# ToyotaResearchInstitute/idto

Hardware: AMD Instinct MI355X
Metric: Gauss-Newton iters/sec (grad+Hessian+solve), mini_cheetah N=40 (higher is better)
Workload: dtype f64; 1 GPU; mini_cheetah (nq=19, nv=18, 9 contact pairs), horizon N=40, dt=0.05, forward differences, one Gauss-Newton iteration per step; parallelism=single GPU

## Files before the change

### idto_amd/csrc/penta_pipe.h

```cpp
#pragma once

#include "kernels.h"
#include "penta_nd.h"
#include "solver_layout.h"

namespace idto_dev {


enum {
  PF_SLOTGEN = 0,
  PF_SLOTGEN2 = 3,
  PF_ROWDONE = 6,
  PF_ROWDONE2 = 9,
  PF_STAGED = 12,
  PF_INITD = 14,
  PF_INITD2 = 16,
  PF_GDONE = 18,
  PF_COPIED = 22,
  PF_COPIED2 = 25,
  PF_ABORT = 28,
  PF_JOINED = 29,
  PF_HIDONE = 30,
  PF_HIDONE2 = 31,
  PF_T0 = 40,
// ... 102 lines not shown
    }
  }
  if constexpr (J + 1 < K) {
    const double m1 = rdlane(t, J + 1);
    xr[J + 1] = __builtin_fma(-m1, xj, xr[J + 1]);
  }
  if constexpr (J == JH) hook();
  if constexpr (J >= 1) {
#pragma unroll
    for (int r = J + 2; r < K; ++r) xr[r] = __builtin_fma(-mu_p[r], xj_p, xr[r]);
    if constexpr ((J & 1) == 0 && J + 1 < K) asm volatile("" ::"v"(mu_p[J]));
  }
  __builtin_amdgcn_sched_barrier(0);
  if constexpr (J + 1 < K) pipe_pivot<K, J + 1, JH>(xr, inv_next, mu, xj, rowp, rawp, slot0, is63, hook, dbg);
}

template <int K, int J, int JH, class Hook, class Need>
__device__ __forceinline__ void pipe_spike_pivot(double (&xr)[K], const double (&mu_p)[K], const double xj_p, const double m1,
                                                 double* __restrict__ rowp, double* __restrict__ fout, const bool store,
                                                 const double* __restrict__ arow, Hook hook, Need need) {
  using G = PipeGeo<K>;
  if constexpr (J == JH) hook();
  if constexpr (J + 2 < K) need(J + 2);
  const double xj = xr[J];
  if constexpr (J + 1 < K) {
    if constexpr (J >= 1) xr[J + 1] = __builtin_fma(-mu_p[J + 1], xj_p, xr[J + 1]);
    xr[J + 1] = __builtin_fma(-m1, xj, xr[J + 1]);
  }
  rowp[J * G::RS] = pipe_setlane<63>(xj, 0x3ff00000, 0);
  __atomic_signal_fence(__ATOMIC_SEQ_CST);
  if (store) __hip_atomic_store(fout + J, xj, __ATOMIC_RELAXED, __HIP_MEMORY_SCOPE_AGENT);
  double mu[K];
  double m1n = 0.0;
  if constexpr (J + 2 < K) {
    const double2* p2 = reinterpret_cast<const double2*>(arow + J * G::RS);
#pragma unroll
    for (int m = (J + 2) / 2; m < (K + 1) / 2; ++m) {
      const double2 v = p2[m];
      mu[2 * m] = v.x;
      if (2 * m + 1 < K) mu[2 * m + 1] = v.y;
    }
    m1n = arow[(J + 1) * G::RS + J + 2];
  }
  if constexpr (J >= 1) {
#pragma unroll
    for (int r = J + 2; r < K; ++r) xr[r] = __builtin_fma(-mu_p[r], xj_p, xr[r]);
  }
  __builtin_amdgcn_sched_barrier(0);
  if constexpr (J + 1 < K) pipe_spike_pivot<K, J + 1, JH>(xr, mu, xj, m1n, rowp, fout, store, arow, hook, need);
}

template <int K>
__device__ __forceinline__ void pipe_read_mult(const double* __restrict__ row, int pos0, double (&mu)[K]) {
  const double2* p2 = reinterpret_cast<const double2*>(row + pos0);
#pragma unroll
  for (int m = 0; m < K / 2; ++m) { const double2 v = p2[m]; mu[2 * m] = v.x; mu[2 * m + 1] = v.y; }
  if (K & 1) mu[K - 1] = row[pos0 + K - 1];
}

__device__ __forceinline__ void pipe_wait_row(const PipeCtl& c, const double* word) {
  pipe_lds_int* hi = (pipe_lds_int*)word + 1;
  int n = 0;
  while ((__builtin_amdgcn_readfirstlane(*hi) & 0x7ff80000) == 0x7ff80000) {
    __builtin_amdgcn_s_sleep(1);
    if (pipe_giveup(c, ++n)) break;
  }
  __atomic_signal_fence(__ATOMIC_SEQ_CST);
}

struct PipeArgs {
  int n, k;
  const double* HA; const double* HB; const double* HC; const double* b;
  double rhs_sign;
  double* x;
  double* Ust; double* Hst; double* Est; double* Dst;
  double* xch; unsigned* flags; unsigned epoch;
  unsigned* status; unsigned fact_id;
  double* fst; int fstride; unsigned long long* frowcnt;
  double* wst;
  double* xjoin_ll;
  double* join_ll;
  const unsigned* asm_ready; int asm_first, asm_rows;
  double* ts;
};

struct PipeAsm {
  int on;
  int nq, nv, rows, first;
  DevProblem P;
  const double* q; const double* terms; const double* v_res; const double* nplus;
  double* g; double* HA; double* HB; double* HC;
  AltSel alt;
  unsigned* ready;
  const double* gate;
  int decide;
  const double* dq;
  const double* dv; const double* dslab; int dslab_stride; double* dcost; int ddiag;
  TrDecideArgs dT; AltSel dalt;
  double* dword; unsigned depoch;
  double* g2; double* HA2; double* HB2; double* HC2;
  const double* curpre;
};
template <bool DEC = false>
__device__ __forceinline__ bool pipe_asm_on(const PipeAsm& F, size_t o, const SpinCtl sc = SpinCtl{nullptr, 0}, int* cur = nullptr) {
  if (!F.on) return false;
  if (DEC && F.decide) {
    double x = 0.0;
    if ((threadIdx.x & 63) == 0) {
      const double* word = at_problem(F.dword, o);
      if (!spin_wait([&] { return tr_ll_try(word, F.depoch, x); }, sc)) x = 1.0;
    }
    const int code = __builtin_amdgcn_readfirstlane((int)x) - 1;
    if (cur) *cur = code >> 1;
    return (code & 1) != 0;
  }
  return !(F.gate && *at_problem(F.gate, o) == 0.0);
}

__device__ __forceinline__ void pipe_decide_role(const PipeAsm& F, const size_t pstride) {
  const size_t o = (size_t)blockIdx.y * pstride, w = o + (size_t)alt_offset(F.dalt, o);
  const DevProblem P = at_problem(F.P, o);
  TrDecideArgs T = F.dT;
  T.state = at_problem(T.state, o); T.out = at_problem(T.out, o); T.q = at_problem(T.q, o);
  T.q_trial = at_problem(T.q_trial, o); T.rows += (size_t)blockIdx.y * T.rows_stride;
  T.part2 = at_problem(T.part2, o);
  if (T.lambda) T.lambda = at_problem(T.lambda, o);
  const double cur_old = T.state[TRS_CUR];
  const bool acc = cost_body<4>(F.nq, F.nv, P, at_problem(F.dq, o), at_problem(F.dv, w), at_problem(F.dslab, w), F.dslab_stride,
                             at_problem(F.dcost, o), F.ddiag, nullptr, nullptr, T);
  if (threadIdx.x == 0) {
    const int cur_new = acc ? (cur_old != 0.0 ? 0 : 1) : (cur_old != 0.0 ? 1 : 0);
    tr_ll_store(at_problem(F.dword, o), (double)(1 + (acc ? 1 : 0) + 2 * cur_new), F.depoch);
  }
}

template <bool DEC = false>
__device__ __forceinline__ void pipe_assemble(double* ts, const unsigned epoch, const size_t pstride, PipeAsm F, const int first_wg,
                                              const SpinCtl sc = SpinCtl{nullptr, 0}) {
  struct { double* ts; unsigned epoch; size_t pstride; } A{ts, epoch, pstride};
  extern __shared__ double lds[];
  const bool decided = DEC && F.decide;
  const int a0 = (int)blockIdx.x - first_wg;
  if (decided && a0 == 0) { pipe_decide_role(F, pstride); return; }
  const int a = decided ? a0 - 1 : a0, i = a >> 2, part = a & 3;
  if (i >= F.rows) return;
  const size_t o = (size_t)blockIdx.y * A.pstride;
  if (!decided && !pipe_asm_on<false>(F, o)) return;
  if (A.ts && threadIdx.x == 0)
    atomicMax(reinterpret_cast<unsigned long long*>(A.ts + first_wg * 64 + 1), (unsigned long long)__double_as_longlong((double)wall_clock64()));
  if (A.ts && a == 4 && threadIdx.x == 0) A.ts[first_wg * 64 + 8] = (double)wall_clock64();
  const size_t w = o + (size_t)(decided ? (((*at_problem(F.curpre, o) != 0.0) != (F.dalt.which != 0)) ? F.dalt.off : 0) : alt_offset(F.alt, o));
  const DevProblem P = at_problem(F.P, o);
  const double* qa = at_problem(decided ? F.dq : F.q, o);
  assemble_terms_row<true>(F.nq, F.nv, P, qa, at_problem(F.terms, w), at_problem(F.v_res, w), at_problem(F.nplus, w),
                           at_problem(decided ? F.g2 : F.g, o), at_problem(decided ? F.HA2 : F.HA, o),
                           at_problem(decided ? F.HB2 : F.HB, o), at_problem(decided ? F.HC2 : F.HC, o), i, part, lds);
  if (A.ts && a == 4 && threadIdx.x == 0) A.ts[first_wg * 64 + 9] = (double)wall_clock64();
  asm volatile("s_waitcnt vmcnt(0)" ::: "memory");
  __syncthreads();
  if (A.ts && a == 4 && threadIdx.x == 0) A.ts[first_wg * 64 + 10] = (double)wall_clock64();
  if (threadIdx.x == 0)
    __hip_atomic_store(at_problem(F.ready, o) + 4 * i + part, A.epoch, __ATOMIC_RELAXED, __HIP_MEMORY_SCOPE_AGENT);
  if (A.ts && threadIdx.x == 0)
    atomicMax(reinterpret_cast<unsigned long long*>(A.ts + first_wg * 64), (unsigned long long)__double_as_longlong((double)wall_clock64()));
  if (decided) {
    if (!pipe_asm_on<true>(F, o, sc)) return;
// ... 562 lines not shown
    for (int t = 0; t < nloc; ++t) {
      const int slot = t % 3;
      const double* row0 = ring + slot * G::SLOT;
      const bool prod = t + 2 < nrows;
      if (!prod && SPK) {
        pipe_wait(ctl, PF_SLOTGEN + slot, t + 1);
        PipeWatch<K, false> watch(row0, true);
        double* xout = (lane >> 2) == 0 ? A.Dst + (size_t)orig(t) * K : A.fst + (size_t)t * A.fstride + 2 * K * ks;
#pragma unroll
        for (int sq = 0; sq < SK; ++sq) {
          watch.need(ctl, (4 * sq + 3 < K ? 4 * sq + 3 : K - 1));
          const int r = 4 * sq + xr4;
          if (lane < 8 && r < K) __hip_atomic_store(xout + r, row0[r * RS + xpos], __ATOMIC_RELAXED, __HIP_MEMORY_SCOPE_AGENT);
        }
      }
      if (prod) {
        pipe_wait(ctl, PF_SLOTGEN + slot, t + 1);
        if (SPK) pipe_wait(ctl, PF_SLOTGEN2 + slot, t + 1);
        PipeWatch<K, SPK> watch(row0, true);
        double* xout = !SPK ? nullptr : (lane >> 2) == 0 ? A.Dst + (size_t)orig(t) * K : A.fst + (size_t)t * A.fstride + 2 * K * ks;
        d4 acc[CT][TT];
#pragma unroll
        for (int tc = 0; tc < CT; ++tc)
#pragma unroll
          for (int tr = 0; tr < TT; ++tr) acc[tc][tr] = d4{0.0, 0.0, 0.0, 0.0};
#pragma unroll
        for (int sq = 0; sq < SK; ++sq) {
          watch.need(ctl, (4 * sq + 3 < K ? 4 * sq + 3 : K - 1));
          if (SPK) {
            const int r = 4 * sq + xr4;
            if (lane < 8 && r < K) __hip_atomic_store(xout + r, row0[r * RS + xpos], __ATOMIC_RELAXED, __HIP_MEMORY_SCOPE_AGENT);
          }
          const double* row = row0 + (4 * sq + fk) * RS;
          double a[TT], bq[CT];
#pragma unroll
          for (int tr = 0; tr < TT; ++tr) a[tr] = row[G::oE + 16 * tr + fl];
#pragma unroll
          for (int tc = 0; tc < CT; ++tc) {
            const int ci = 16 * tc + fl;
            bq[tc] = row[ci < G::KE + 2 ? G::oRE + ci : G::oF + ci - (G::KE + 2)];
          }
#pragma unroll
          for (int tc = 0; tc < CT; ++tc)
#pragma unroll
            for (int tr = 0; tr < TT; ++tr) acc[tc][tr] = __builtin_amdgcn_mfma_f64_16x16x4f64(a[tr], bq[tc], acc[tc][tr], 0, 0, 0);
        }
        double* gout = gbuf + (t & 1) * G::NGC * GS;
#pragma unroll
        for (int tc = 0; tc < CT; ++tc)
#pragma unroll
          for (int tr = 0; tr < TT; ++tr)
#pragma unroll
            for (int rg = 0; rg < 4; ++rg) {
              const int r = 16 * tr + fk + 4 * rg, ci = 16 * tc + fl;
              if (r < K && ci < NCG) gout[ci * GS + r] = acc[tc][tr][rg];
            }
        pipe_post(ctl, PF_GDONE + (t & 1), t + 1);
      }
      if (SPK) {
        asm volatile("s_waitcnt vmcnt(0)" ::: "memory");
        if (lane == 0) __hip_atomic_fetch_add(A.frowcnt + t, 2ull, __ATOMIC_RELAXED, __HIP_MEMORY_SCOPE_AGENT);
      }
    }
  }
  __syncthreads();
  if (tid == 0 && ctl.f[PF_ABORT] != 0 && cfg.spin.word) {
    __hip_atomic_store(cfg.spin.word, cfg.spin.id, __ATOMIC_RELAXED, __HIP_MEMORY_SCOPE_SYSTEM);
    __hip_atomic_fetch_add(cfg.spin.word + 1, 1u, __ATOMIC_RELAXED, __HIP_MEMORY_SCOPE_SYSTEM);
  }
  chain_ts(cfg, 2);
}


__device__ __forceinline__ double pipe_half_sum(double v) {
  const unsigned lo = (unsigned)__double2loint(v), hi = (unsigned)__double2hiint(v);
  const auto a = __builtin_amdgcn_permlane32_swap(lo, lo, false, false);
  const auto b = __builtin_amdgcn_permlane32_swap(hi, hi, false, false);
  return __hiloint2double((int)b[0], (int)a[0]) + __hiloint2double((int)b[1], (int)a[1]);
}

template <int K, bool SPK>
__device__ __forceinline__ bool pipe_backward_fits(const PipeLds& L, int nloc) { return nloc * PipeBack<K, SPK>::BS + 4 * PipeBack<K, SPK>::KE + 2 <= L.xall; }

template <int K, bool SPK, bool WGLOB = false>
__device__ __forceinline__ void pipe_backward(const PipeArgs& A, const ChainCfg& cfg, const PipeLds& L) {
  extern __shared__ double lds[];
  using B = PipeBack<K, SPK && !WGLOB>;
  constexpr int ks = ldl_ks(K), KE = B::KE, YS = B::YS, KS2 = K * ks;
  const int tid = threadIdx.x, lane = tid & 63, wave = __builtin_amdgcn_readfirstlane(tid >> 6), nwaves = blockDim.x >> 6;
  const bool mirror = cfg.mirror != 0, producer = cfg.producer != 0;
  const int nloc = cfg.nloc, m_split = cfg.m_split, k = A.k;
  auto orig = [&](int il) { const int o = mirror ? cfg.base - il : cfg.base + il; return o < 0 ? 0 : o; };
  double* xb = lds + nloc * B::BS;
  double* dump = xb + 4 * KE;
  auto solve = [&](const double* Us, double (&xr)[K]) __attribute__((always_inline)) {
    constexpr int NP = (K + 1) / 2;
    double2 ub[2][NP];
    auto loadu = [&](int r, double2 (&u)[NP]) __attribute__((always_inline)) {
      const double2* u2 = reinterpret_cast<const double2*>(Us + r * ks);
#pragma unroll
      for (int m = (r + 1) / 2; m < NP; ++m) u[m] = u2[m];
    };
    if (K >= 2) loadu(K - 2, ub[0]);
#pragma unroll
    for (int q = 0; q < K - 1; ++q) {
      const int r = K - 2 - q;
      if (r >= 1) loadu(r - 1, ub[(q + 1) & 1]);
      asm volatile("" ::: "memory");
      double a0 = 0.0, a1 = 0.0;
#pragma unroll
      for (int m = (r + 1) / 2; m < NP; ++m) {
        const double2 u = ub[q & 1][m];
        if (2 * m > r) a0 = __builtin_fma(u.x, xr[2 * m], a0);
        if (2 * m + 1 < K) a1 = __builtin_fma(u.y, xr[2 * m + 1], a1);
      }
      xr[r] -= a0 + a1;
    }
  };
  auto do_pass = [&](const int il, const int pass, const bool stage) __attribute__((always_inline)) {
    const bool partner = WGLOB && pass == 1;
    if (partner) {
      spin_wait([&] { return __hip_atomic_load(cfg.wp_frowcnt + il, __ATOMIC_RELAXED, __HIP_MEMORY_SCOPE_AGENT) >= cfg.frowtarget; }, cfg.spin);
      (void)__hip_atomic_load(cfg.wp_frowcnt + il, __ATOMIC_ACQUIRE, __HIP_MEMORY_SCOPE_AGENT);
    }
    const int op = cfg.wp_mirror ? cfg.wp_base - il : cfg.wp_base + il;
    const int o = partner ? (op < 0 ? 0 : op) : orig(il);
    double* slot = lds + il * B::BS;
    double* Us = partner ? lds + L.W + 2 * KE + 2 + wave * KS2 : slot + ((pass && !WGLOB) ? B::oW : B::oYZ);
    constexpr int NU = (KS2 + 63) / 64;
    double uv[NU];
    if (stage) {
#pragma unroll
      for (int t = 0; t < NU; ++t) uv[t] = A.Ust[(size_t)o * KS2 + (lane + 64 * t < KS2 ? lane + 64 * t : 0)];
    }
    const double dinv = (lane < K) ? A.Dst[(size_t)o * K + lane] : 0.0;
    double xr[K];
    double* dst = dump;
    int dstride = 0;
    if (pass == 0) {
      const double* src = (lane < K) ? A.Hst + (size_t)o * KS2 + lane : A.Est + (size_t)o * KS2 + (lane < 2 * K ? lane - K : 0);
      const double mg = lane < 2 * K ? 1.0 : 0.0, mc = lane == 2 * K ? 1.0 : 0.0;
#pragma unroll
      for (int r = 0; r < K; ++r) xr[r] = src[r * ks] * mg + (rdlane(dinv, r) * lds[L.xall + (il + 2) * ks + r]) * mc;
      if (lane < 2 * K) { dst = slot + B::oYZ + (lane < K ? lane : KE + lane - K); dstride = YS; }
      else if (lane == 2 * K) { dst = slot + B::oC; dstride = 1; }
      else if ((K & 1) && lane <= 2 * K + 2) { dst = slot + B::oYZ + (lane == 2 * K + 1 ? K : KE + K); dstride = YS; }
    } else {
      const double* fsrc = (WGLOB ? cfg.wp_fst : A.fst) + (size_t)il * A.fstride + (size_t)(lane < 2 * K ? lane : 0) * ks;
      const double mf = lane < 2 * K ? 1.0 : 0.0;
#pragma unroll
      for (int r = 0; r < K; ++r) xr[r] = (rdlane(dinv, r) * fsrc[r]) * mf;
      if (WGLOB) {
        if (lane < 2 * K) { dst = cfg.wp_wst + (size_t)il * A.fstride + (size_t)lane * ks; dstride = 1; }
      } else {
        if (lane < 2 * K) { dst = slot + B::oW + (lane < K ? lane : KE + lane - K); dstride = YS; }
        else if ((K & 1) && lane <= 2 * K + 1) { dst = slot + B::oW + (lane == 2 * K ? K : KE + K); dstride = YS; }
      }
    }
    if (stage) {
#pragma unroll
      for (int t = 0; t < NU; ++t) if (lane + 64 * t < KS2) Us[lane + 64 * t] = uv[t];
    }
    __atomic_signal_fence(__ATOMIC_SEQ_CST);
    solve(Us, xr);
    __atomic_signal_fence(__ATOMIC_SEQ_CST);
    if (partner) {
      double* Tw = Us;
      double* wrow_dst = cfg.wp_wst + (size_t)il * A.fstride;
#pragma unroll
      for (int half = 0; half < 2; ++half) {
        if (lane >= half * K && lane < half * K + K) {
#pragma unroll
          for (int r = 0; r < K; ++r) Tw[(lane - half * K) * ks + r] = xr[r];
        }
        __atomic_signal_fence(__ATOMIC_SEQ_CST);
#pragma unroll
        for (int t = 0; t < NU; ++t)
          if (lane + 64 * t < KS2) __hip_atomic_store(wrow_dst + half * KS2 + lane + 64 * t, Tw[lane + 64 * t], __ATOMIC_RELAXED, __HIP_MEMORY_SCOPE_AGENT);
        __atomic_signal_fence(__ATOMIC_SEQ_CST);
      }
      asm volatile("s_waitcnt vmcnt(0)" ::: "memory");
      if (lane == 0) __hip_atomic_store(cfg.wrow + il, A.epoch, __ATOMIC_RELAXED, __HIP_MEMORY_SCOPE_AGENT);
    } else {
#pragma unroll
      for (int r = 0; r < K; ++r) dst[r * dstride] = xr[r];
    }
  };
  if (WGLOB) {
    const int ws = (cfg.wp_wst && wave < cfg.wp_waves) ? cfg.wp_waves : 0, wn = ws ? cfg.wp_nloc : 0;
    auto ask = [&](int il) { return il < wn ? __hip_atomic_load(cfg.wp_frowcnt + il, __ATOMIC_RELAXED, __HIP_MEMORY_SCOPE_AGENT) : 0ull; };
    auto there = [&](unsigned long long cnt) { return __builtin_amdgcn_readfirstlane(cnt >= cfg.frowtarget ? 1 : 0); };
    int own = wave, wt = wave;
    int ready = there(ask(wt));
    while (own < nloc || wt < wn) {
      if (wt < wn && (ready || own >= nloc)) {
        const unsigned long long nxt = ask(wt + ws);
        do_pass(wt, 1, true);
        wt += ws;
        ready = there(nxt);
      } else {
        const unsigned long long nxt = ask(wt);
        do_pass(own, 0, true);
        own += nwaves;
        ready = there(nxt);
      }
    }
  } else {
    for (int task = wave; task < (SPK ? 2 : 1) * nloc; task += nwaves) {
      const int pass = task >= nloc ? 1 : 0;
      do_pass(task - pass * nloc, pass, true);
    }
  }
  __syncthreads();
  chain_ts(cfg, 3);
  if (cfg.ts && tid == 0) cfg.ts[6] = (double)wall_clock64();
  if (WGLOB && cfg.fst) {
    const int nt = blockDim.x;
    const int pidx = (tid < nloc * K) ? tid : 0, pil = pidx / K, pr = pidx - pil * K;
    const int qidx = (tid + nt < nloc * K) ? tid + nt : 0, qil = qidx / K, qr = qidx - qil * K;
    double f[2 * K], f2[2 * K];
    {
      spin_wait([&] { return __hip_atomic_load(cfg.wrow + pil, __ATOMIC_RELAXED, __HIP_MEMORY_SCOPE_AGENT) == A.epoch; }, cfg.spin);
      __builtin_amdgcn_fence(__ATOMIC_ACQUIRE, "agent");
      const double* F = A.wst + (size_t)pil * A.fstride + pr;
#pragma unroll
      for (int c = 0; c < 2 * K; ++c) f[c] = F[c * ks];
#pragma unroll
      for (int c = 0; c < 2 * K; ++c) asm volatile("" : "+v"(f[c]));
      if (cfg.ts && tid == 0) cfg.ts[7] = (double)wall_clock64();
      spin_wait([&] { return __hip_atomic_load(cfg.wrow + qil, __ATOMIC_RELAXED, __HIP_MEMORY_SCOPE_AGENT) == A.epoch; }, cfg.spin);
      __builtin_amdgcn_fence(__ATOMIC_ACQUIRE, "agent");
      const double* F2 = A.wst + (size_t)qil * A.fstride + qr;
#pragma unroll
      for (int c = 0; c < 2 * K; ++c) f2[c] = F2[c * ks];
#pragma unroll
      for (int c = 0; c < 2 * K; ++c) asm volatile("" : "+v"(f2[c]));
    }
    double* xs = lds + L.W;
    if (tid < 2 * KE) {
      const int half = tid / KE, r = tid - half * KE;
      xs[tid] = (r < K) ? ll_load(cfg.xsep_ll + 2 * ((mirror ? half : 1 - half) * K + r), A.epoch, cfg.spin) : 0.0;
    }
    __syncthreads();
    if (tid < nloc * K) {
      double a0 = 0.0, a1 = 0.0;
#pragma unroll
      for (int c = 0; c < K; ++c) { a0 = __builtin_fma(f[c], xs[c], a0); a1 = __builtin_fma(f[K + c], xs[KE + c], a1); }
      lds[pil * B::BS + B::oC + pr] -= a0 + a1;
    }
    if (tid + nt < nloc * K) {
      double a0 = 0.0, a1 = 0.0;
#pragma unroll
      for (int c = 0; c < K; ++c) { a0 = __builtin_fma(f2[c], xs[c], a0); a1 = __builtin_fma(f2[K + c], xs[KE + c], a1); }
      lds[qil * B::BS + B::oC + qr] -= a0 + a1;
    }
    __syncthreads();
  }
  if (!WGLOB && SPK && cfg.fst) {
    double* xs = lds + L.W;
    if (tid < 2 * KE) {
      const int half = tid / KE, r = tid - half * KE;
      xs[tid] = (r < K) ? ll_load(cfg.xsep_ll + 2 * ((mirror ? half : 1 - half) * K + r), A.epoch, cfg.spin) : 0.0;
    }
    __syncthreads();
    for (int il = wave; il < nloc; il += nwaves) {
      if (lane < K) {
        const double2* w2 = reinterpret_cast<const double2*>(lds + il * B::BS + B::oW + lane * YS);
        const double2* x2 = reinterpret_cast<const double2*>(xs);
        double a0 = 0.0, a1 = 0.0;
#pragma unroll
        for (int m = 0; m < KE; ++m) { const double2 w = w2[m], x = x2[m]; a0 = __builtin_fma(w.x, x.x, a0); a1 = __builtin_fma(w.y, x.y, a1); }
        lds[il * B::BS + B::oC + lane] -= a0 + a1;
      }
    }
    __syncthreads();
  }
  if (wave != 0) return;
  if (cfg.ts && tid == 0) cfg.ts[21] = (double)wall_clock64();
  const int hf = lane >> 5, r_ = lane & 31, rr = r_ < K ? r_ : 0;
  static_assert(K <= 32, "one row per lane of a half-wavefront");
  for (int c = lane; c < 4 * KE; c += 64) xb[c] = 0.0;
  if (cfg.two && producer) {
    if (lane < K) {
      xb[(nloc & 3) * KE + lane] = ll_load(A.xjoin_ll + 2 * (K + lane), A.epoch, cfg.spin);
      xb[((nloc + 1) & 3) * KE + lane] = ll_load(A.xjoin_ll + 2 * lane, A.epoch, cfg.spin);
    }
  }
  double M0[KE], M1[KE], c0 = 0.0, c1 = 0.0;
  auto fetch = [&](int il, double (&M)[KE], double& c) __attribute__((always_inline)) {
    const double2* y2 = reinterpret_cast<const double2*>(lds + il * B::BS + B::oYZ + rr * YS + hf * KE);
#pragma unroll
    for (int m = 0; m < KE / 2; ++m) { const double2 a = y2[m]; M[2 * m] = a.x; M[2 * m + 1] = a.y; }
    c = lds[il * B::BS + B::oC + rr];
  };
  auto row = [&](int il, const double (&M)[KE], const double c, double (&Mn)[KE], double& cn) __attribute__((always_inline)) {
    const double2* xv = reinterpret_cast<const double2*>(xb + ((il + 1 + hf) & 3) * KE);
    double x[KE];
#pragma unroll
    for (int m = 0; m < KE / 2; ++m) { const double2 a = xv[m]; x[2 * m] = a.x; x[2 * m + 1] = a.y; }
    if (il >= 1) fetch(il - 1, Mn, cn);
    double a0 = 0.0, a1 = 0.0;
#pragma unroll
    for (int m = 0; m < KE / 2; ++m) { a0 = __builtin_fma(M[2 * m], x[2 * m], a0); a1 = __builtin_fma(M[2 * m + 1], x[2 * m + 1], a1); }
    const double part = a0 + a1;
    const double v = c - pipe_half_sum(part);
    if (lane < K) {
      xb[(il & 3) * KE + lane] = v;
      if (lane < k) A.x[(size_t)orig(il) * k + lane] = v;
      if (cfg.two && !producer && il >= m_split) ll_store(A.xjoin_ll + 2 * ((il - m_split) * K + lane), v, A.epoch);
    }
    __atomic_signal_fence(__ATOMIC_SEQ_CST);
  };
  if (nloc > 0) fetch(nloc - 1, M0, c0);
  if (cfg.ts && tid == 0) cfg.ts[22] = (double)wall_clock64();
  for (int il = nloc - 1; il >= 0; il -= 2) {
    row(il, M0, c0, M1, c1);
    if (il >= 1) row(il - 1, M1, c1, M0, c0);
  }
  chain_ts(cfg, 4);
}

template <int K>
__device__ void chain_recursion_tail(int n, int k, double* x, double* Ust, double* Hst, double* Est, double* Dst,
                                     const ChainCfg& cfg, unsigned epoch, int xall_off) {
  extern __shared__ double lds[];
  using B = PipeBack<K, false>;
  constexpr int ks = ldl_ks(K);
  const int tid = threadIdx.x, nloc = cfg.nloc;
  PipeLds L = {};
  L.xall = cfg.lds_doubles - (nloc + 2) * ks;
  L.W = nloc * B::BS + 4 * B::KE + 2;
  {
    double keep[4];
#pragma unroll
    for (int j = 0; j < 4; ++j) keep[j] = (tid + 256 * j < (nloc + 2) * ks) ? lds[xall_off + tid + 256 * j] : 0.0;
    __syncthreads();
#pragma unroll
    for (int j = 0; j < 4; ++j) if (tid + 256 * j < (nloc + 2) * ks) lds[L.xall + tid + 256 * j] = keep[j];
    __syncthreads();
  }
  PipeArgs P = {};
  P.n = n; P.k = k; P.x = x; P.Ust = Ust; P.Hst = Hst; P.Est = Est; P.Dst = Dst; P.epoch = epoch;
  P.fst = const_cast<double*>(cfg.fst); P.fstride = cfg.fstride; P.wst = cfg.wst; P.xjoin_ll = cfg.xjoin_ll;
  pipe_backward<K, true, true>(P, cfg, L);
}

template <int K, bool DEC = false>
__global__ void __launch_bounds__(512) penta_pipe_kernel(NdArgs A, PipeAsm F) {
  if (blockIdx.x >= 5) {
    pipe_assemble<DEC>(A.ts, A.epoch, A.pstride, F, 5, SpinCtl{A.status + 2 * gridDim.y, A.fact_id});
    return;
  }
  {
    const size_t o = (size_t)blockIdx.y * A.pstride;
    A.HA = at_problem(A.HA, o); A.HB = at_problem(A.HB, o); A.HC = at_problem(A.HC, o); A.b = at_problem(A.b, o);
    A.x = at_problem(A.x, o); A.Ust = at_problem(A.Ust, o); A.Hst = at_problem(A.Hst, o); A.Est = at_problem(A.Est, o);
    A.Dst = at_problem(A.Dst, o); A.xch = at_problem(A.xch, o); A.flags = at_problem(A.flags, o);
    A.rowcnt = at_problem(A.rowcnt, o); A.ndbuf = at_problem(A.ndbuf, o);
    A.spin = SpinCtl{A.status + 2 * gridDim.y, A.fact_id};
    A.status += 2 * blockIdx.y;
  }
  const int role = blockIdx.x;
  if (role == A.debug_skip_role) return;
  const bool asm_on = pipe_asm_on<DEC>(F, (size_t)blockIdx.y * A.pstride, A.spin);
  if (DEC && F.decide && asm_on) {
    const size_t o = (size_t)blockIdx.y * A.pstride, qq0 = (size_t)F.first * F.nq * F.nq;
    A.HA = at_problem(F.HA2, o) + qq0; A.HB = at_problem(F.HB2, o) + qq0; A.HC = at_problem(F.HC2, o) + qq0;
    A.b = at_problem(F.g2, o) + (size_t)F.first * F.nq;
  }
  if (role == 4) {
    A.asm_ready = asm_on ? at_problem(F.ready, (size_t)blockIdx.y * A.pstride) : nullptr;
    A.asm_first = F.first;
    A.wt_rows = 1;
    nd_separator<K, false>(A);
    return;
  }
  const NdBuf B = nd_layout(K);
  ChainCfg c = {};
  c.two = 1;
  c.dbg_slot = role;
  c.ts = A.ts ? A.ts + role * 64 : nullptr;
  c.spin = A.spin;
  int pair;
  if (role == 0) { c.mirror = 0; c.producer = 1; c.base = 0; c.nloc = A.j1; pair = 0; }
  else if (role == 1) { c.mirror = 1; c.producer = 1; c.base = A.n - 1; c.nloc = A.n - A.j2 - 2; pair = 1; }
  else {
    const int w = role - 2;
    c.mirror = (w == 0); c.producer = 0;
    c.base = (w == 0) ? A.s - 1 : A.s + 2;
    c.m_split = (w == 0) ? A.s - A.j1 - 2 : A.j2 - A.s - 2;
    c.nloc = c.m_split + 2;
    pair = w;
    c.fst = A.ndbuf + B.fst + (size_t)w * ND_MAXROWS * B.frow; c.fstride = B.frow;
    c.frowcnt = A.rowcnt + (2 + w) * ND_MAXROWS; c.frowtarget = (A.rowtarget / A.rowunit) * 3ull;
    c.xsep = A.ndbuf + B.xsep; c.sepflag = A.flags + 4;
    c.xsep_ll = A.ndbuf + B.ll;
  }
  PipeArgs P;
  P.n = A.n; P.k = A.k; P.HA = A.HA; P.HB = A.HB; P.HC = A.HC; P.b = A.b; P.rhs_sign = A.rhs_sign; P.x = A.x;
  P.Ust = A.Ust; P.Hst = A.Hst; P.Est = A.Est; P.Dst = A.Dst;
  P.xch = A.xch + (size_t)pair * A.xch_pair; P.flags = A.flags + 2 * pair; P.epoch = A.epoch;
  P.status = A.status; P.fact_id = A.fact_id;
  P.fst = const_cast<double*>(c.fst); P.fstride = c.fstride;
  P.frowcnt = role >= 2 ? A.rowcnt + (2 + role - 2) * ND_MAXROWS : nullptr;
  P.ts = c.ts;
  P.xjoin_ll = A.ndbuf + B.ll + (1 + pair) * 4 * K;
  P.join_ll = A.ndbuf + B.joinll + (size_t)pair * B.joinll_pair;
  P.asm_ready = asm_on ? at_problem(F.ready, (size_t)blockIdx.y * A.pstride) : nullptr;
  P.asm_first = F.first; P.asm_rows = F.rows;
  const bool spike = role >= 2;
  const PipeLds L = pipe_layout<K>(A.n, spike);
  if (spike) pipe_forward<K, true>(P, c, L);
  else pipe_forward<K, false>(P, c, L);
  const bool recursion = K > 8 && !A.debug_pipe_tail && pipe_backward_fits<K, true>(pipe_layout<K>(A.n, true), max(A.s - A.j1, A.j2 - A.s)) &&
                         pipe_backward_fits<K, false>(pipe_layout<K>(A.n, false), max(A.j1, A.n - A.j2 - 2));
  if (recursion) {
    if (spike) pipe_backward<K, true>(P, c, L);
    else pipe_backward<K, false>(P, c, L);
    return;
  }
  if (threadIdx.x >= 256) return;
  penta_ldl_tail<K, 256>(A.n, A.k, 1, A.x, A.Ust, A.Hst, A.Est, A.Dst, nullptr, c, P.xch, P.flags, A.epoch, L.xall, 1,
                         L.W, c.nloc + (c.producer ? 2 : 0));
}

}
```

### idto_amd/csrc/solver_layout.h

```cpp
#pragma once

#ifdef __HIPCC__
#define IDTO_LAYOUT_HD __host__ __device__
#else
#define IDTO_LAYOUT_HD
#endif

#define IDTO_LDL_KERNELS(X) \
  X(2, false, 1) X(3, false, 1) X(5, false, 1) X(19, false, 1) X(23, false, 2) X(8, true, 1) X(16, true, 1) X(24, true, 2) \
  X(30, true, 2) X(29, false, 2) X(4, false, 1) X(32, true, 3)
#define IDTO_ND_KERNELS(X) X(2) X(3) X(5) X(19) X(23) X(29) X(8)
#define IDTO_PIPE_KERNELS(X) X(2) X(3) X(5) X(19)
#define IDTO_PIPE_DEC_KERNELS(X) X(5) X(19)
#define IDTO_BAND_KERNELS(X) X(6) X(9) X(12) X(15)
#define IDTO_APPLY_KERNELS(X) X(2) X(3) X(5) X(8) X(16) X(19) X(23) X(24) X(32)
#define IDTO_FUSED_KERNELS(X) X(2, 2, false, 1) X(3, 3, false, 1) X(3, 5, false, 1) X(3, 19, false, 1) X(4, 23, false, 2)
#define IDTO_SMALL_KERNELS(X) X(1, 6, 6, false) X(5, 9, 9, false) X(1, 6, 6, true) X(5, 9, 9, true) X(1, 6, 9, true) X(5, 9, 12, true)

namespace idto_dev {

enum SolverFamily { FAM_LDL, FAM_ND, FAM_PIPE, FAM_PIPE_DEC, FAM_BAND, FAM_APPLY };
constexpr bool SolverInstantiated(SolverFamily f, int v) {
#define IDTO_X1(K) || v == K
#define IDTO_X3(K, PD, GW) || v == K
// ... 83 lines not shown


struct BandLds { int m, lim, nb, pad, tcols, bcols, T, Bm, Dt, Db, D0, J, end; };
constexpr int BAND_FRONT = 32;
IDTO_LAYOUT_HD inline BandLds band_layout(int M, int W) {
  BandLds L;
  L.m = ((M - W) / 2 + W / 2) / W * W;
  L.lim = L.m + W;
  L.nb = M - W - L.m;
  L.pad = (W - L.nb % W) % W;
  L.tcols = BAND_FRONT + L.lim + 2 * W + 1;
  L.bcols = BAND_FRONT + L.pad + L.nb + 2 * W + 1;
  int o = 0;
  L.T = o; o += L.tcols * 16;
  L.Bm = o; o += L.bcols * 16;
  L.Dt = o; o += L.tcols;
  L.Db = o; o += L.bcols;
  L.D0 = o; o += M + (M & 1);
  L.J = o; o += W * 16;
  L.end = o;
  return L;
}


template <int K>
struct PipeGeo {
  static constexpr int KE = K + (K & 1);
  static constexpr int KR = 4 * ((K + 3) / 4);
  static constexpr int oS = 0, oH = KE, oE = 2 * KE, oy = 3 * KE, oF = 3 * KE + 2;
  static constexpr int od = oF + 2 * K;
  static constexpr int og = od + 1;
  static constexpr int oi = og + 1;
  static constexpr int odump = oi + 1;
  static constexpr int oz = odump + 8;
  static constexpr int oRH = oz + 1 + ((oz + 1) & 1), oRE = oRH + KE, oRy = oRE + KE;
  static constexpr int used = oRy + 1;
  static constexpr int RS = ((used + 15) / 32) * 32 + 16;
  static constexpr int SLOT = KR * RS;
  static constexpr int GS = ldl_ks(K);
  static constexpr int NCX = 3 * K + 1;
  static constexpr int NGC = KE + 2 + 2 * K;
  static_assert(3 * K <= 61, "main wavefront: 3K + 1 columns and the lane that publishes d");
  static_assert(RS >= used && RS % 32 == 16, "row stride");
};

template <int K>
constexpr int pipe_rlo() { return K >= 17 ? 16 : (K >= 3 ? (((K + 1) / 2 + 1) & ~1) : K); }
template <int K>
constexpr bool pipe_mfma_follow() { return K >= 17; }
constexpr int PIPE_HPC = 48, PIPE_HS = 18, PIPE_HPN = (PIPE_HPC + 1) * PIPE_HS;

struct PipeLds {
  int ring, stage, gbuf, xhi, hp, jbuf, xall, W, flags, end;
};
template <int K>
IDTO_LAYOUT_HD inline PipeLds pipe_layout(int n, bool spike) {
  using G = PipeGeo<K>;
  PipeLds L;
  int o = 0;
  L.ring = o; o += 3 * G::SLOT;
  L.stage = o; o += 2 * G::NCX * G::GS + 2;
  L.gbuf = o; o += 2 * G::NGC * G::GS;
  {
    constexpr int NHI = K - pipe_rlo<K>();
    L.xhi = o; o += (G::NCX + (spike ? 2 * K : 0) + 1) * (NHI + (NHI & 1)) + 2;
  }
  L.hp = o; o += pipe_mfma_follow<K>() ? (spike ? 2 : 1) * PIPE_HPN : 0;
  (void)n;
  L.jbuf = o; o += spike ? (3 * K + 2) * G::KE : 0;
  L.xall = o; o += (ND_MAXROWS + 2) * G::GS;
  L.W = o; o += 2 * G::KE + 2;
  L.flags = o; o += 32;
  L.end = o;
  return L;
}

template <int K, bool SPK>
struct PipeBack {
  static constexpr int KE = K + (K & 1), YS0 = 2 * KE > ldl_ks(K) ? 2 * KE : ldl_ks(K), YS = YS0 + (YS0 % 8 == 0 ? 2 : 0);
  static constexpr int oYZ = 0, oW = K * YS, oC = oW + (SPK ? K * YS : 0), BS = oC + KE;
};

template <int K>
IDTO_LAYOUT_HD inline int pipe_recursion_tail_fits(int lds_doubles, int nloc_joiner, int nloc_producer) {
  using B = PipeBack<K, false>;
  constexpr int ks = ldl_ks(K);
  const int nloc = nloc_joiner > nloc_producer ? nloc_joiner : nloc_producer;
  if (!(nloc_joiner * B::BS + 6 * B::KE + 4 <= lds_doubles - (nloc_joiner + 2) * ks && (nloc + 2) * ks <= 4 * 256 &&
        nloc_joiner * K <= 2 * 256))
    return 0;
  for (int w = 4; w >= 1; w >>= 1)
    if (nloc_producer * B::BS + 6 * B::KE + 4 + w * K * ks <= lds_doubles - (nloc_producer + 2) * ks) return w;
  return 0;
}


IDTO_LAYOUT_HD constexpr int gn_small_fold_doubles(int N, int K) { return 26 * (N + 1) * K + 18 * (N + 1) + 32; }

IDTO_LAYOUT_HD inline int gn_small_doubles(int N, int K, int fast_n, int KK = 0) {
  const int E = 1 + 3 * K;
  if (KK > K) return gn_small_doubles(N, K, fast_n) + 3 * (N + 1) * KK * KK + (N + 1) * KK;
  return 2 * (N + 1) * K + N * K + 3 * N * E + N * E * K + K * K + 3 * N * K * K + 5 * K + (K & 1) + fast_n + (fast_n & 1) +
         3 * (N + 1) * K * K + 3 * (N + 1) * K + 2 * K * K + (K * K & 1) + K + 2 +
         5 * K + (K & 1) + (3 * N + 2) * (K + 1) + 2 * (N + 1) + 2 + 24;
}

}
```

Baseline: 13010 GN iters/s.

## Replace serial producer back-substitution tail with MFMA closed-form affine recursion

Adds a closed-form tail for non-spike producer blocks. Before the join values arrive, it builds affine maps from each local row's solution to the two join rows, using f64 MFMA tiles spread across all waves. Once the join values land, every thread finishes its own output with a single dot product, replacing a serial row-by-row back-substitution on one wavefront. The spike path is also changed to overlap the W-correction with wave 0's start of the recursion, fetching M0 early and using an LDS barrier. The cost is extra LDS and MFMA work on the critical path before the join, plus more synchronization complexity.

```diff
diff --git a/idto_amd/csrc/penta_pipe.h b/idto_amd/csrc/penta_pipe.h
--- a/idto_amd/csrc/penta_pipe.h
+++ b/idto_amd/csrc/penta_pipe.h
@@ -208,6 +208,7 @@
   double* join_ll;
   const unsigned* asm_ready; int asm_first, asm_rows;
   double* ts;
+  int closed_tail;
 };
 
 struct PipeAsm {
@@ -936,6 +937,95 @@
 template <int K, bool SPK>
 __device__ __forceinline__ bool pipe_backward_fits(const PipeLds& L, int nloc) { return nloc * PipeBack<K, SPK>::BS + 4 * PipeBack<K, SPK>::KE + 2 <= L.xall; }
 
+template <int K>
+__device__ __forceinline__ bool pipe_closed_fits(const PipeLds& L, int nloc) { return PipeClosed<K>::end(nloc) <= L.xall; }
+
+template <int K>
+__device__ __forceinline__ void pipe_closed_tail() {
+  extern __shared__ double lds[];
+  using B = PipeBack<K, false>;
+  using C = PipeClosed<K>;
+  using d4 = __attribute__((ext_vector_type(4))) double;
+  constexpr int KE = B::KE, YS = B::YS, TS = C::TS, NC = C::NC;
+  constexpr int TT = (K + 15) / 16, CT = (NC + 15) / 16, SK = 2 * KE / 4;
+  static_assert(2 * K <= 64, "a lane per component of the two join rows");
+  const int tid = threadIdx.x, lane = tid & 63, wave = __builtin_amdgcn_readfirstlane(tid >> 6), nt = blockDim.x, nwaves = nt >> 6;
+  const int xall = pipe_layout<K>(0, false).xall;
+  const unsigned long long* par = reinterpret_cast<const unsigned long long*>(lds + xall + C::PAR);
+  const int nloc = __builtin_amdgcn_readfirstlane((int)(unsigned)par[5]);
+  double* x = reinterpret_cast<double*>(par[0]);
+  const double* xjoin_ll = reinterpret_cast<const double*>(par[1]);
+  const SpinCtl spin = {reinterpret_cast<unsigned*>(par[2]), (unsigned)(par[4] >> 32)};
+  double* ts = reinterpret_cast<double*>(par[3]);
+  const unsigned epoch = (unsigned)par[4];
+  const int k = (int)(unsigned)(par[5] >> 32), base = (int)(unsigned)par[6], mirror = (int)(unsigned)(par[6] >> 32);
+  auto orig = [&](int il) { const int o = mirror ? base - il : base + il; return o < 0 ? 0 : o; };
+  double* T = lds + C::base(nloc);
+  for (int idx = tid; idx < 2 * C::SLOT; idx += nt) {
+    const int h = idx / C::SLOT, r = (idx - h * C::SLOT) / TS, n = idx - h * C::SLOT - r * TS;
+    T[nloc * C::SLOT + idx] = (n == h * KE + r) ? 1.0 : 0.0;
+  }
+  __syncthreads();
+  const int fl = lane & 15, fk = lane >> 4;
+  for (int il = nloc - 1; il >= 0; --il) {
+    const double* yz = lds + il * B::BS + B::oYZ;
+    const double* cc = lds + il * B::BS + B::oC;
+    double* Ti = T + il * C::SLOT;
+    for (int tile = wave; tile < TT * CT; tile += nwaves) {
+      const int tr = tile / CT, tc = tile - tr * CT;
+      const int ar = 16 * tr + fl < K ? 16 * tr + fl : K - 1;
+      const int bn = 16 * tc + fl < NC ? 16 * tc + fl : NC - 1;
+      double a[SK], b[SK];
+#pragma unroll
+      for (int sq = 0; sq < SK; ++sq) {
+        const int p = 4 * sq + fk, h = p >= KE ? 1 : 0, pr = p - h * KE;
+        a[sq] = yz[ar * YS + p];
+        const double t = Ti[(1 + h) * C::SLOT + (pr < K ? pr : K - 1) * TS + bn];
+        b[sq] = pr < K ? t : 0.0;
+      }
+      d4 acc = {0.0, 0.0, 0.0, 0.0};
+#pragma unroll
+      for (int sq = 0; sq < SK; ++sq) acc = __builtin_amdgcn_mfma_f64_16x16x4f64(a[sq], b[sq], acc, 0, 0, 0);
+#pragma unroll
+      for (int rg = 0; rg < 4; ++rg) {
+        const int r = 16 * tr + fk + 4 * rg, n = 16 * tc + fl;
+        if (r < K && n < NC) Ti[r * TS + n] = (n == NC - 1 ? cc[r] : 0.0) - acc[rg];
+      }
+    }
+    __syncthreads();
+  }
+  if (ts && tid == 0) ts[21] = (double)wall_clock64();
+  if (wave * 64 >= nloc * K) return;
+  double* xj = lds + xall + wave * 2 * KE;
+  if (lane < 2 * KE) xj[lane] = 0.0;
+  __atomic_signal_fence(__ATOMIC_SEQ_CST);
+  const int idx0 = wave * 64 + lane, idx = idx0 < nloc * K ? idx0 : 0, il = idx / K, r = idx - il * K;
+  double g[2 * KE];
+  {
+    const double2* g2 = reinterpret_cast<const double2*>(T + il * C::SLOT + r * TS);
+#pragma unroll
+    for (int m = 0; m < KE; ++m) { const double2 v = g2[m]; g[2 * m] = v.x; g[2 * m + 1] = v.y; }
+  }
+  const double chat = T[il * C::SLOT + r * TS + NC - 1];
+  if (lane < 2 * K) {
+    const int h = lane >= K ? 1 : 0, c = lane - h * K;
+    xj[h * KE + c] = ll_load(xjoin_ll + 2 * ((1 - h) * K + c), epoch, spin);
+  }
+  __atomic_signal_fence(__ATOMIC_SEQ_CST);
+  if (ts && tid == 0) ts[22] = (double)wall_clock64();
+  const double2* x2 = reinterpret_cast<const double2*>(xj);
+  double a0 = 0.0, a1 = 0.0, a2 = 0.0, a3 = 0.0;
+#pragma unroll
+  for (int m = 0; m < KE; m += 2) {
+    const double2 u = x2[m], v = x2[m + 1];
+    a0 = __builtin_fma(g[2 * m], u.x, a0); a1 = __builtin_fma(g[2 * m + 1], u.y, a1);
+    a2 = __builtin_fma(g[2 * m + 2], v.x, a2); a3 = __builtin_fma(g[2 * m + 3], v.y, a3);
+  }
+  const double v = chat + ((a0 + a1) + (a2 + a3));
+  if (idx0 < nloc * K && r < k) x[(size_t)orig(il) * k + r] = v;
+  if (ts && tid == 0) ts[4] = (double)wall_clock64();
+}
+
 template <int K, bool SPK, bool WGLOB = false>
 __device__ __forceinline__ void pipe_backward(const PipeArgs& A, const ChainCfg& cfg, const PipeLds& L) {
   extern __shared__ double lds[];
@@ -1068,6 +1158,19 @@
   __syncthreads();
   chain_ts(cfg, 3);
   if (cfg.ts && tid == 0) cfg.ts[6] = (double)wall_clock64();
+  if constexpr (!WGLOB && !SPK) {
+    if (A.closed_tail) {
+      if (tid == 0) {
+        unsigned long long* par = reinterpret_cast<unsigned long long*>(lds + L.xall + PipeClosed<K>::PAR);
+        par[0] = (unsigned long long)A.x; par[1] = (unsigned long long)A.xjoin_ll; par[2] = (unsigned long long)cfg.spin.word;
+        par[3] = (unsigned long long)cfg.ts; par[4] = (unsigned long long)A.epoch | ((unsigned long long)cfg.spin.id << 32);
+        par[5] = (unsigned long long)(unsigned)nloc | ((unsigned long long)(unsigned)k << 32);
+        par[6] = (unsigned long long)(unsigned)cfg.base | ((unsigned long long)(unsigned)cfg.mirror << 32);
+      }
+      __syncthreads();
+      return;
+    }
+  }
   if (WGLOB && cfg.fst) {
     const int nt = blockDim.x;
     const int pidx = (tid < nloc * K) ? tid : 0, pil = pidx / K, pr = pidx - pil * K;
@@ -1110,43 +1213,59 @@
     }
     __syncthreads();
   }
-  if (!WGLOB && SPK && cfg.fst) {
+  const int hf = lane >> 5, r_ = lane & 31, rr = r_ < K ? r_ : 0;
+  static_assert(K <= 32, "one row per lane of a half-wavefront");
+  double M0[KE], M1[KE], c0 = 0.0, c1 = 0.0;
+  auto fetch_m = [&](int il, double (&M)[KE]) __attribute__((always_inline)) {
+    const double2* y2 = reinterpret_cast<const double2*>(lds + il * B::BS + B::oYZ + rr * YS + hf * KE);
+#pragma unroll
+    for (int m = 0; m < KE / 2; ++m) { const double2 a = y2[m]; M[2 * m] = a.x; M[2 * m + 1] = a.y; }
+  };
+  auto fetch = [&](int il, double (&M)[KE], double& c) __attribute__((always_inline)) {
+    fetch_m(il, M);
+    c = lds[il * B::BS + B::oC + rr];
+  };
+  constexpr bool early = !WGLOB && SPK;
+  if constexpr (early) {
     double* xs = lds + L.W;
+    if (wave == 0) {
+      for (int c = lane; c < 4 * KE; c += 64) xb[c] = 0.0;
+      if (nloc > 0) fetch_m(nloc - 1, M0);
+#pragma unroll
+      for (int m = 0; m < KE; ++m) asm volatile("" : "+v"(M0[m]));
+    }
     if (tid < 2 * KE) {
       const int half = tid / KE, r = tid - half * KE;
       xs[tid] = (r < K) ? ll_load(cfg.xsep_ll + 2 * ((mirror ? half : 1 - half) * K + r), A.epoch, cfg.spin) : 0.0;
     }
     __syncthreads();
-    for (int il = wave; il < nloc; il += nwaves) {
-      if (lane < K) {
-        const double2* w2 = reinterpret_cast<const double2*>(lds + il * B::BS + B::oW + lane * YS);
+    for (int t = 2 * wave + hf; t < nloc; t += 2 * nwaves) {
+      const int il = nloc - 1 - t;
+      if (r_ < K) {
+        const double2* w2 = reinterpret_cast<const double2*>(lds + il * B::BS + B::oW + r_ * YS);
         const double2* x2 = reinterpret_cast<const double2*>(xs);
         double a0 = 0.0, a1 = 0.0;
 #pragma unroll
         for (int m = 0; m < KE; ++m) { const double2 w = w2[m], x = x2[m]; a0 = __builtin_fma(w.x, x.x, a0); a1 = __builtin_fma(w.y, x.y, a1); }
-        lds[il * B::BS + B::oC + lane] -= a0 + a1;
-      }
-    }
-    __syncthreads();
-  }
-  if (wave != 0) return;
+        lds[il * B::BS + B::oC + r_] -= a0 + a1;
+      }
+    }
+    __atomic_signal_fence(__ATOMIC_SEQ_CST);
+  }
+  if (wave != 0) {
+    if constexpr (early) lds_barrier();
+    return;
+  }
   if (cfg.ts && tid == 0) cfg.ts[21] = (double)wall_clock64();
-  const int hf = lane >> 5, r_ = lane & 31, rr = r_ < K ? r_ : 0;
-  static_assert(K <= 32, "one row per lane of a half-wavefront");
-  for (int c = lane; c < 4 * KE; c += 64) xb[c] = 0.0;
+  if constexpr (!early) {
+    for (int c = lane; c < 4 * KE; c += 64) xb[c] = 0.0;
+  }
   if (cfg.two && producer) {
     if (lane < K) {
       xb[(nloc & 3) * KE + lane] = ll_load(A.xjoin_ll + 2 * (K + lane), A.epoch, cfg.spin);
       xb[((nloc + 1) & 3) * KE + lane] = ll_load(A.xjoin_ll + 2 * lane, A.epoch, cfg.spin);
     }
   }
-  double M0[KE], M1[KE], c0 = 0.0, c1 = 0.0;
-  auto fetch = [&](int il, double (&M)[KE], double& c) __attribute__((always_inline)) {
-    const double2* y2 = reinterpret_cast<const double2*>(lds + il * B::BS + B::oYZ + rr * YS + hf * KE);
-#pragma unroll
-    for (int m = 0; m < KE / 2; ++m) { const double2 a = y2[m]; M[2 * m] = a.x; M[2 * m + 1] = a.y; }
-    c = lds[il * B::BS + B::oC + rr];
-  };
   auto row = [&](int il, const double (&M)[KE], const double c, double (&Mn)[KE], double& cn) __attribute__((always_inline)) {
     const double2* xv = reinterpret_cast<const double2*>(xb + ((il + 1 + hf) & 3) * KE);
     double x[KE];
@@ -1165,11 +1284,22 @@
     }
     __atomic_signal_fence(__ATOMIC_SEQ_CST);
   };
-  if (nloc > 0) fetch(nloc - 1, M0, c0);
-  if (cfg.ts && tid == 0) cfg.ts[22] = (double)wall_clock64();
-  for (int il = nloc - 1; il >= 0; il -= 2) {
-    row(il, M0, c0, M1, c1);
-    if (il >= 1) row(il - 1, M1, c1, M0, c0);
+  if constexpr (early) {
+    if (nloc > 0) c0 = lds[(nloc - 1) * B::BS + B::oC + rr];
+    if (cfg.ts && tid == 0) cfg.ts[22] = (double)wall_clock64();
+    if (nloc > 0) row(nloc - 1, M0, c0, M1, c1);
+    lds_barrier();
+    for (int il = nloc - 2; il >= 0; il -= 2) {
+      row(il, M1, c1, M0, c0);
+      if (il >= 1) row(il - 1, M0, c0, M1, c1);
+    }
+  } else {
+    if (nloc > 0) fetch(nloc - 1, M0, c0);
+    if (cfg.ts && tid == 0) cfg.ts[22] = (double)wall_clock64();
+    for (int il = nloc - 1; il >= 0; il -= 2) {
+      row(il, M0, c0, M1, c1);
+      if (il >= 1) row(il - 1, M1, c1, M0, c0);
+    }
   }
   chain_ts(cfg, 4);
 }
@@ -1262,15 +1392,19 @@
   P.join_ll = A.ndbuf + B.joinll + (size_t)pair * B.joinll_pair;
   P.asm_ready = asm_on ? at_problem(F.ready, (size_t)blockIdx.y * A.pstride) : nullptr;
   P.asm_first = F.first; P.asm_rows = F.rows;
+  P.closed_tail = 0;
   const bool spike = role >= 2;
   const PipeLds L = pipe_layout<K>(A.n, spike);
   if (spike) pipe_forward<K, true>(P, c, L);
   else pipe_forward<K, false>(P, c, L);
-  const bool recursion = K > 8 && !A.debug_pipe_tail && pipe_backward_fits<K, true>(pipe_layout<K>(A.n, true), max(A.s - A.j1, A.j2 - A.s)) &&
+  const bool recursion = K > 8 && A.debug_pipe_tail != 1 && pipe_backward_fits<K, true>(pipe_layout<K>(A.n, true), max(A.s - A.j1, A.j2 - A.s)) &&
                          pipe_backward_fits<K, false>(pipe_layout<K>(A.n, false), max(A.j1, A.n - A.j2 - 2));
   if (recursion) {
+    const int np = max(A.j1, A.n - A.j2 - 2);
+    P.closed_tail = !spike && A.debug_pipe_tail != 2 && pipe_closed_fits<K>(pipe_layout<K>(A.n, false), np) && np * K <= (int)blockDim.x;
     if (spike) pipe_backward<K, true>(P, c, L);
     else pipe_backward<K, false>(P, c, L);
+    if (P.closed_tail) pipe_closed_tail<K>();
     return;
   }
   if (threadIdx.x >= 256) return;
diff --git a/idto_amd/csrc/solver_layout.h b/idto_amd/csrc/solver_layout.h
--- a/idto_amd/csrc/solver_layout.h
+++ b/idto_amd/csrc/solver_layout.h
@@ -189,6 +189,15 @@
 };
 
 template <int K>
+struct PipeClosed {
+  using B = PipeBack<K, false>;
+  static constexpr int KE = B::KE, NC = 2 * KE + 1, TS0 = 2 * KE + 2, TS = TS0 + (TS0 % 8 == 0 ? 2 : 0), SLOT = K * TS;
+  static constexpr int PAR = 8 * 2 * KE;
+  IDTO_LAYOUT_HD static constexpr int base(int nloc) { return nloc * B::BS + 4 * KE + 2; }
+  IDTO_LAYOUT_HD static constexpr int end(int nloc) { return base(nloc) + (nloc + 2) * SLOT; }
+};
+
+template <int K>
 IDTO_LAYOUT_HD inline int pipe_recursion_tail_fits(int lds_doubles, int nloc_joiner, int nloc_producer) {
   using B = PipeBack<K, false>;
   constexpr int ks = ldl_ks(K);
```

Result: faster. 13230 GN iters/s (median of 6 runs) (+1.7%).
